# ArtoriasAbyssslayer/HashModNFFBanks-IDR

Hardware: AMD Instinct MI355X
Metric: rays/sec fwd+bwd (hash+SDF MLP) (higher is better)
Workload: dtype f32; 1 GPU; DTU-shaped synthetic uniform-sphere rays, MultiResHash L=16 T=2^19 F=2 (BASELINE.json configs[1]), full IDR training step (forward + IDRLoss + backward + clip + Adam), weights held at the geometric initialisation (lr = 0): the SURVEY.md 8(d) workload; grid_config=C2, rays_per_gpu=2048, global_rays=2048, parallelism=single GPU, world=1, ranks_seen=1, step=HIP-graph captured static-shape step

## Files before the change

### hashmodnffbanks_idr_amd/_lib.py

```python
import ctypes as C
import os

import torch

_PKG = os.path.dirname(os.path.abspath(__file__))
LIB_PATH = os.environ.get("HM_LIB_PATH") or os.path.join(_PKG, "libhashmod.so")
_lib = None

_p = C.c_void_p
_i64 = C.c_int64
_int = C.c_int

SIGNATURES = {
    "hm_version": (_int, []),
    "hm_last_error": (C.c_char_p, []),
    "hm_device_count": (_int, []),
    "hm_grid_desc_create": (_int, [_int, _int, _p, _p, _p, C.POINTER(_p)]),
    "hm_grid_desc_destroy": (None, [_p]),
    "hm_grid_embed_dim": (_int, [_p]),
    "hm_corner_ids": (_int, [_p, _int, _p, _i64, _p, _p, _p]),
    "hm_diag_gather_calib": (_int, [_p, _i64, _i64, _int, _int, _p, _p]),
    "hm_diag_mfma_f32_stream": (_int, [_int, _int, _p, _p]),
    "hm_encode_fwd": (_int, [_p, _p, _i64, _p, _p, _p, _i64, _int, _p]),
    "hm_encode_workspace_bytes": (_i64, [_p, _i64]),
# ... 60 lines not shown
    "hm_gemm_f32_det": (_int, [_int, _int, _i64, _i64, _i64, _p, _i64, _p, _i64, _p, _p, _i64, _int, _p, _i64, _p]),
    "hm_gemm_f32_group_tn_det_workspace_bytes": (_i64, [_p, _int]),
    "hm_gemm_f32_group_tn_det": (_int, [_p, _int, _p, _i64, _p]),
    "hm_gemm_f32_group_tn_add": (_int, [_p, _int, _p]),
    "hm_gemm_f32_group_tn_add_det_workspace_bytes": (_i64, [_p, _int]),
    "hm_gemm_f32_group_tn_add_det": (_int, [_p, _int, _p, _i64, _p]),
    "hm_colsum_det_workspace_bytes": (_i64, [_i64, _i64]),
    "hm_colsum_det": (_int, [_p, _i64, _i64, _i64, _p, _p, _i64, _p]),
    "hm_colsum_acc_det": (_int, [_p, _i64, _i64, _i64, _p, _p, _i64, _p]),
    "hm_colsum_acc_multi_det_workspace_bytes": (_i64, [_p, _int]),
    "hm_colsum_acc_multi_det": (_int, [_p, _int, _p, _i64, _p]),
    "hm_encode_bwd_table_sorted_tracked": (_int, [_p, _p, _p, _i64, _int, _p, _i64, _p, _p, _p, _p, _p, _i64, _p]),
    "hm_gemm_f32_ep": (_int, [_int, _int, _i64, _i64, _i64, _p, _i64, _p, _i64, _p, _p, _i64, _p, _p]),
    "hm_gemm_f32": (_int, [_int, _int, _i64, _i64, _i64, _p, _i64, _p, _i64, _p, _p, _i64, _int, _p]),
    "hm_diag_gemm_plan": (_int, [_int, _int, _i64, _i64, _i64, _p, _i64, _p, _i64, _int, _int, _p]),
    "hm_mc_workspace_bytes": (_i64, [_i64, _i64, _i64]),
    "hm_mc_count": (_int, [_p, _i64, _i64, _i64, _i64, _i64, _i64, C.c_float, _p, _i64, _p, _p]),
    "hm_mc_emit": (_int, [_p, _i64, _i64, _i64, _i64, _i64, _i64, C.c_float, _p, _p, _i64, _i64, _i64, _p, _p, _p,
                          _p]),
    "hm_mcs_points_bricks": (_int, [_p, _i64, _p, _p, _p, _i64, _i64, _i64, _p, _p, _p]),
    "hm_mcs_points_index": (_int, [_p, _i64, _p, _p, _p, _i64, _i64, _i64, _p, _p, _p]),
    "hm_mcs_status": (_int, [_p, _i64, _p, C.c_float, _p, _p]),
    "hm_mcs_workspace_bytes": (_i64, [_i64]),
    "hm_mcs_count": (_int, [_p, _i64, _p, C.c_float, _p, _i64, _p, _p]),
    "hm_mcs_emit": (_int, [_p, _i64, _p, _p, C.c_float, _p, _p, _i64, _i64, _i64, _p, _p, _p, _p, _p, _p]),
    "hm_mesh_cc_labels": (_int, [_p, _i64, _i64, _p, _p, _p]),
    "hm_mesh_cc_face_stats": (_int, [_p, _p, _i64, _i64, _p, _p, _p, _p]),
    "hm_mesh_cc_sums_workspace_bytes": (_i64, [_i64]),
    "hm_mesh_cc_sums": (_int, [_p, _i64, _i64, _p, _p, _p, _i64, _p, _p, _p, _i64, _p, _p]),
    "hm_mesh_moments_workspace_bytes": (_i64, [_i64]),
# ... 247 lines not shown
```

### hashmodnffbanks_idr_amd/csrc/hm_gemm.hip

```cpp
#include "hm_common.h"

namespace {

typedef float f32x16 __attribute__((ext_vector_type(16)));


struct GemmArgs {
    const float *A, *B, *bias;
    float *C;
    int32_t M, N, K;
    int32_t transA, transB;
    int32_t vec_out;
    int64_t lda, ldb, ldc;
    int32_t k_chunk;
    int32_t atomic;
    int32_t vecA, vecB;
    int32_t nrecA, nrecB;
    hm_gemm_epilogue ep;
};

template <int ROWS>
__device__ __forceinline__ int lds_slot(int kg, int row) {
    return (kg * ROWS + (row ^ (kg & 7))) * 4;
}
// ... 420 lines not shown
        const int kg = 2 * oo + h;
        xa[oo] = *reinterpret_cast<const float4 *>(as + lds_slot<AROWS>(kg, arow));
        xb[oo] = *reinterpret_cast<const float4 *>(bs + lds_slot<64>(kg, brow));
    }
}
__device__ __forceinline__ void pipe_mfma_oct(const float4 &a, const float4 &b, f32x16 &c) {
    c = __builtin_amdgcn_mfma_f32_32x32x2f32(a.x, b.x, c, 0, 0, 0);
    c = __builtin_amdgcn_mfma_f32_32x32x2f32(a.y, b.y, c, 0, 0, 0);
    c = __builtin_amdgcn_mfma_f32_32x32x2f32(a.z, b.z, c, 0, 0, 0);
    c = __builtin_amdgcn_mfma_f32_32x32x2f32(a.w, b.w, c, 0, 0, 0);
}


template <bool AKC, bool BKC, bool EP, int WM = 2, bool PART = false, bool KT = false, int ADD = 0>
__device__ __forceinline__ void gemm_pipe2_body(const GemmArgs &g, int bx, int by, int bz, const GemmAddend *ad = nullptr) {
    constexpr int BM = 32 * WM, BN = 64, BK = kPipeBK, NT = 256 * WM, NTB = 512, PER = BM * BK / 4 / NT, KG = BK / 4,
                  OCT = BK / 8 / 2;
    static_assert(PER == 1 && BN * BK / 4 / NTB == 1, "one k-group per thread and operand");
    __shared__ __align__(16) float As_static[ADD ? 1 : 2][ADD ? 4 : BK * BM];
    __shared__ __align__(16) float Bs_static[ADD ? 1 : 2][ADD ? 4 : BK * BN];
    float (*As)[BK * BM], (*Bs)[BK * BN];
    if constexpr (ADD != 0) {
        extern __shared__ __align__(16) float hm_pipe_dyn_lds[];
        As = reinterpret_cast<float (*)[BK * BM]>(hm_pipe_dyn_lds);
        Bs = reinterpret_cast<float (*)[BK * BN]>(hm_pipe_dyn_lds + 2 * BK * BM);
    } else {
        As = As_static;
        Bs = Bs_static;
    }
    const int tid = threadIdx.x;
    const int wave = tid >> 6, lane = tid & 63;
    const int kpart = wave / (2 * WM), wsub = wave % (2 * WM);
    const int wm = wsub >> 1, wn = wsub & 1;
    const int j = lane & 31, h = lane >> 5;
    const int m0 = bx * BM, n0 = by * BN;
    const int kbeg = bz * g.k_chunk;
    const int stages = g.k_chunk / BK;
#ifdef HM_GEMM_PHASE_PROBE
    unsigned long long probe_wait = 0;
#endif
    HM_GEMM_STAMP(0);

    const __amdgpu_buffer_rsrc_t rsA = __builtin_amdgcn_make_buffer_rsrc(const_cast<float *>(g.A), 0, g.nrecA, 0x00020000);
    const __amdgpu_buffer_rsrc_t rsB = __builtin_amdgcn_make_buffer_rsrc(const_cast<float *>(g.B), 0, g.nrecB, 0x00020000);
    int va[PER], vb[PER];
    int kla[PER], klb[PER];
#pragma unroll
    for (int i = 0; i < PER; ++i) {
        const int e = tid + NT * i;
        const int eb = (tid % NTB) + NTB * i;
        const int am = min(m0 + (AKC ? e / KG : e % BM), g.M - 1), bn = min(n0 + (BKC ? eb / KG : eb % BN), g.N - 1);
        va[i] = (int)(4 * (AKC ? (int64_t)am * g.lda + kbeg + (e % KG) * 4
                               : (int64_t)(kbeg + (e / BM) * 4) * g.lda + am));
        vb[i] = (int)(4 * (BKC ? (int64_t)bn * g.ldb + kbeg + (eb % KG) * 4
                               : (int64_t)(kbeg + (eb / BN) * 4) * g.ldb + bn));
        if (KT) {
            kla[i] = g.K - kbeg - (e % KG) * 4;
            klb[i] = g.K - kbeg - (eb % KG) * 4;
        }
    }
    __amdgpu_buffer_rsrc_t rsA2 = rsA, rsB2 = rsB;
    int va2[PER], vb2[PER];
    int sa2 = 0, sb2 = 0, lda24 = 0, ldb24 = 0;
    if constexpr (ADD != 0) {
        static_assert(!AKC && !BKC && !KT, "addends are built for the grouped TN form");
        rsA2 = __builtin_amdgcn_make_buffer_rsrc(const_cast<float *>(ad->A2), 0, ad->nrecA2, 0x00020000);
        rsB2 = __builtin_amdgcn_make_buffer_rsrc(const_cast<float *>(ad->B2), 0, ad->nrecB2, 0x00020000);
        lda24 = 4 * ad->lda2;
        ldb24 = 4 * ad->ldb2;
        sa2 = BK * lda24;
        sb2 = BK * ldb24;
#pragma unroll
        for (int i = 0; i < PER; ++i) {
            const int e = tid + NT * i;
            const int eb = (tid % NTB) + NTB * i;
            const int am = min(m0 + e % BM, g.M - 1), bn = min(n0 + eb % BN, g.N - 1);
            va2[i] = 4 * ((kbeg + (e / BM) * 4 - ad->a_k0) * ad->lda2 + am);
            vb2[i] = 4 * ((kbeg + (eb / BN) * 4 - ad->b_k0) * ad->ldb2 + bn);
        }
    }
#define HM_PIPE_MASK(S_, N_)                                                                        \
    do {                                                                                            \
        if (KT) {                                                                                   \
            pipe_mask_tail<AKC, PER>(ra##N_, kla, (S_) * BK);                                       \
            pipe_mask_tail<BKC, PER>(rb##N_, klb, (S_) * BK);                                       \
        }                                                                                           \
        if constexpr ((ADD & 1) != 0) pipe_add<PER>(ra##N_, qa##N_);                                \
        if constexpr ((ADD & 2) != 0) pipe_add<PER>(rb##N_, qb##N_);                                \
    } while (0)
    const bool stage_b = NT == NTB || tid < NTB;
    const int sa = 4 * (AKC ? BK : BK * (int)g.lda), sb = 4 * (BKC ? BK : BK * (int)g.ldb);
    const int lda4 = 4 * (int)g.lda, ldb4 = 4 * (int)g.ldb;
    f32x16 acc, acc2;
#pragma unroll
    for (int r = 0; r < 16; ++r) acc[r] = acc2[r] = 0.0f;
    static_assert(kPipeD == 4, "the stage macro below is written out for a 4-deep ring (8-deep measured no faster)");
    float4 ra0[PER], ra1[PER], ra2[PER], ra3[PER], rb0[PER], rb1[PER], rb2[PER], rb3[PER];
    float4 qa0[PER], qa1[PER], qa2[PER], qa3[PER], qb0[PER], qb1[PER], qb2[PER], qb3[PER];
    float4 opa0[OCT], opa1[OCT], opb0[OCT], opb1[OCT];
#define HM_PIPE_FETCH(S_, F_)                                                                       \
    do {                                                                                            \
        const int sc_ = min((S_), stages - 1);  \
        pipe_fetch_buf<AKC, PER>(rsA, va, sc_ * sa, lda4, ra##F_);                                  \
        pipe_fetch_buf<BKC, PER>(rsB, vb, sc_ * sb, ldb4, rb##F_);                                  \
        if constexpr ((ADD & 1) != 0) pipe_fetch_add<PER>(rsA2, va2, sc_ * sa2, lda24, qa##F_);     \
        if constexpr ((ADD & 2) != 0) pipe_fetch_add<PER>(rsB2, vb2, sc_ * sb2, ldb24, qb##F_);     \
    } while (0)
    HM_PIPE_FETCH(0, 0);
    HM_PIPE_FETCH(1, 1);
    HM_PIPE_FETCH(2, 2);
    HM_PIPE_MASK(0, 0);
    store_tile<BM, BK, NT>(As[0], AKC, tid, ra0);
    if (stage_b) store_tile<BN, BK, NTB>(Bs[0], BKC, tid, rb0);
    __syncthreads();
    HM_GEMM_STAMP(1);
    pipe_read_ops<OCT, BM>(As[0], Bs[0], wm * 32 + j, wn * 32 + j, h + 4 * kpart, opa0, opb0);
#define HM_PIPE_STAGE(S_, F_, N_, C_, X_, NB_)                                                      \
    do {                                                                                            \
        HM_PIPE_FETCH((S_) + kPipeD - 1, F_);                                                       \
        pipe_mfma_oct(opa##C_[0], opb##C_[0], acc);                                                 \
        HM_PIPE_MASK((S_) + 1, N_);                                                                 \
// ... 71 lines not shown
template <bool AKC, bool BKC, bool EP>
__global__ __launch_bounds__(512, 4) void gemm_f32_pipe2_ktail_kernel(GemmArgs g) {
    gemm_pipe2_body<AKC, BKC, EP, 2, false, true>(g, blockIdx.x, blockIdx.y, blockIdx.z);
}
template <bool AKC, bool BKC, bool EP>
__global__ __launch_bounds__(768, 3) void gemm_f32_pipe2_m96_ktail_kernel(GemmArgs g) {
    gemm_pipe2_body<AKC, BKC, EP, 3, false, true>(g, blockIdx.x, blockIdx.y, blockIdx.z);
}
template <bool AKC, bool BKC>
__global__ __launch_bounds__(512, 4) void gemm_f32_pipe2_part_kernel(GemmArgs g) {
    gemm_pipe2_body<AKC, BKC, false, 2, true>(g, blockIdx.x, blockIdx.y, blockIdx.z);
}
template <bool AKC, bool BKC>
__global__ __launch_bounds__(768, 3) void gemm_f32_pipe2_m96_part_kernel(GemmArgs g) {
    gemm_pipe2_body<AKC, BKC, false, 3, true>(g, blockIdx.x, blockIdx.y, blockIdx.z);
}

struct GemmGroupEntry {
    const float *A, *B;
    float *C;
    int64_t lda, ldb, ldc;
    int32_t M, N, k_chunk, tiles_m, tiles_n, split;
};
struct GemmGroupTable {
    GemmGroupEntry e[HM_GEMM_GROUP_MAX];
    int32_t start[HM_GEMM_GROUP_MAX + 1];
    int32_t n;
};
struct GemmGroupAddTable {
    GemmGroupTable t;
// ... 129 lines not shown
}

static bool gemm_vec_out(const GemmArgs &g, bool part) {
    auto ok = [](const void *p, int64_t ld) { return (reinterpret_cast<uintptr_t>(p) & 15u) == 0 && ld % 4 == 0; };
    if ((g.atomic && !part) || g.N % 4 != 0 || !ok(g.C, g.ldc)) return false;
    const hm_gemm_epilogue &e = g.ep;
    if (e.mode == HM_EPI_NONE) return true;
    const bool masked = e.mode == HM_EPI_S1MUL || e.mode == HM_EPI_RELUMASK;
    const bool has_z = masked || e.mode == HM_EPI_ADJOINT;
    if (!ok(e.out1, e.ld1) || (masked && e.nz % 4 != 0)) return false;
    if (has_z && (!ok(e.z, e.ldz) || (e.g && !ok(e.g, e.ldg)))) return false;
    if (e.mode == HM_EPI_ADJOINT && (!ok(e.out2, e.ld2) || (e.out3 && !ok(e.out3, e.ld3)))) return false;
    return true;
}

static int64_t gemm_det_bytes(const GemmPlan &P, int64_t M, int64_t N) {
    return P.split > 1 ? 4 * P.split * M * N : 0;
}

static int launch_part_reduce(const GemmReduceTable &t, hipStream_t st) {
    if (t.end == 0) return HM_OK;
    HM_CHECK_ARG((t.end + 255) / 256 < (1ll << 31), "hm_gemm_f32_det: too many elements for one reduce launch");
    hipLaunchKernelGGL(gemm_part_reduce_kernel, dim3((unsigned)((t.end + 255) / 256)), dim3(256), 0, st, t);
    return HM_OK;
}

static int gemm_impl(int transA, int transB, int64_t M, int64_t N, int64_t K, const float *A, int64_t lda,
                     const float *B, int64_t ldb, const float *bias, float *C, int64_t ldc, int accumulate,
                     const hm_gemm_epilogue *ep, void *stream, bool det = false, float *ws = nullptr,
                     int64_t ws_bytes = 0) {
    HM_CHECK_ARG(M >= 0 && N >= 0 && K >= 0, "hm_gemm_f32: negative dimension");
    HM_CHECK_ARG(M < (1ll << 31) && N < (1ll << 31) && K < (1ll << 31), "hm_gemm_f32: dimension too large");
    if (M == 0 || N == 0) return HM_OK;
    HM_CHECK_ARG(C != nullptr || (ep && ep->mode != HM_EPI_NONE), "hm_gemm_f32: C is NULL");
    HM_CHECK_ARG(K == 0 || (A && B), "hm_gemm_f32: NULL operand");
    HM_CHECK_ARG(lda >= (transA ? M : K) && ldb >= (transB ? K : N) && (!C || ldc >= N), "hm_gemm_f32: leading dimension");
    GemmArgs g;
    g.ep = hm_gemm_epilogue{};
    if (ep && ep->mode != HM_EPI_NONE) {
        HM_CHECK_ARG(!accumulate, "hm_gemm_f32_ep: an epilogue cannot be combined with accumulate");
        HM_CHECK_ARG(ep->mode >= HM_EPI_SOFTPLUS && ep->mode <= HM_EPI_RELUMASK, "hm_gemm_f32_ep: unknown epilogue mode");
        const bool masked = ep->mode == HM_EPI_S1MUL || ep->mode == HM_EPI_RELUMASK;
        HM_CHECK_ARG(ep->out1 && ep->ld1 >= (masked ? ep->nz : N), "hm_gemm_f32_ep: out1");
        if (ep->mode != HM_EPI_SOFTPLUS && ep->mode != HM_EPI_RELU) {
            const int64_t nzc = masked ? ep->nz : N;
// ... 6 lines not shown
        }
        g.ep = *ep;
    }
    g.A = A; g.B = B; g.bias = bias; g.C = C;
    g.M = (int)M; g.N = (int)N; g.K = (int)K;
    g.transA = transA; g.transB = transB;
    g.lda = lda; g.ldb = ldb; g.ldc = ldc;
    const GemmPlan P = gemm_plan(transA, transB, M, N, K, A, lda, B, ldb, g.ep.mode != HM_EPI_NONE);
    g.vecA = P.vecA ? 1 : 0;
    g.vecB = P.vecB ? 1 : 0;
    const bool big = P.big, m96 = P.m96, pipe_ok = P.pipe_ok;
    const int64_t bm = P.bm, bn = P.bn, split = P.split;
    g.nrecA = (int32_t)(P.bytesA < 0x7fffffff ? P.bytesA : 0x7fffffff);
    g.nrecB = (int32_t)(P.bytesB < 0x7fffffff ? P.bytesB : 0x7fffffff);
    g.k_chunk = (int)P.k_chunk;
    const bool part = det && split > 1;
    if (part) {
        HM_CHECK_ARG(ws != nullptr && ws_bytes >= gemm_det_bytes(P, M, N), "hm_gemm_f32_det: workspace too small");
        g.C = ws;
        g.ldc = N;
    }
    g.atomic = (accumulate || split > 1) ? 1 : 0;
    g.vec_out = gemm_vec_out(g, part) ? 1 : 0;
    if (split > 1 && !accumulate && !part) {
        hipLaunchKernelGGL(zero_window_kernel, dim3((unsigned)((M * N + 255) / 256)), dim3(256), 0, as_stream(stream),
                           C, ldc, M, N);
    }
    dim3 grid((unsigned)((M + bm - 1) / bm), (unsigned)((N + bn - 1) / bn), (unsigned)split);
    HM_CHECK_ARG(grid.y <= 65535u && grid.z <= 65535u, "hm_gemm_f32: N or split too large for one launch");
    hipStream_t st = as_stream(stream);
// ... 66 lines not shown
    HM_CHECK_ARG(M >= 0 && N >= 0 && K >= 0, "hm_diag_gemm_plan: negative dimension");
    *info = hm_gemm_plan_info{};
    if (M == 0 || N == 0) return HM_OK;
    const GemmPlan P = gemm_plan(transA, transB, M, N, K, A, lda, B, ldb, has_epilogue != 0);
    info->kernel = P.big ? HM_GEMM_KERNEL_BIG
                 : P.pipe_ok ? (P.m96 ? HM_GEMM_KERNEL_PIPE96 : HM_GEMM_KERNEL_PIPE64) : HM_GEMM_KERNEL_GENERIC;
    info->k_tail = P.k_tail ? 1 : 0;
    info->vec_a = P.vecA ? 1 : 0;
    info->vec_b = P.vecB ? 1 : 0;
    info->part = (deterministic && P.split > 1) ? 1 : 0;
    info->split = P.split;
    info->k_chunk = P.k_chunk;
    return HM_OK;
}

int hm_gemm_f32_det(int transA, int transB, int64_t M, int64_t N, int64_t K, const float *A, int64_t lda,
                    const float *B, int64_t ldb, const float *bias, float *C, int64_t ldc, int accumulate,
                    void *workspace, int64_t workspace_bytes, void *stream) {
    return gemm_impl(transA, transB, M, N, K, A, lda, B, ldb, bias, C, ldc, accumulate, nullptr, stream, true,
                     static_cast<float *>(workspace), workspace_bytes);
}

}

template <class Item>
static int group_tn(const char *who, const Item *items, int n_items, bool det, float *ws, int64_t ws_bytes,
                    void *stream, bool run, int64_t *need) {
    constexpr bool ADD = std::is_same<Item, hm_gemm_group_add_item>::value;
    HM_CHECK_ARG(n_items >= 0 && (n_items == 0 || items), std::string(who) + ": bad argument");
    *need = 0;
// ... 167 lines not shown
}

#ifdef HM_GEMM_PHASE_PROBE
HM_API int hm_gemm_probe_read(unsigned long long *out, int n) {
    return hipMemcpyFromSymbol(out, HIP_SYMBOL(hm_gemm_probe_ts), sizeof(unsigned long long) * (size_t)(n < 8 ? n : 8)) == hipSuccess ? 0 : -1;
}
#endif

int hm_gemm_f32_ep(int transA, int transB, int64_t M, int64_t N, int64_t K, const float *A, int64_t lda,
                   const float *B, int64_t ldb, const float *bias, float *C, int64_t ldc,
                   const hm_gemm_epilogue *ep, void *stream) {
    HM_CHECK_ARG(ep != nullptr, "hm_gemm_f32_ep: epilogue is NULL");
    return gemm_impl(transA, transB, M, N, K, A, lda, B, ldb, bias, C, ldc, 0, ep, stream);
}

}
```

### hashmodnffbanks_idr_amd/mlp_grad.py

```python
import math

import torch

from . import ops
from .ops import (EPI_ADJOINT, EPI_RELU, EPI_RELUMASK, EPI_S1MUL, EPI_SOFTPLUS, _softplus_call, colsum_into_multi, gemm,
                  gemm_ep, gemm_group_tn, gemm_group_tn_add)

_SQRT2 = math.sqrt(2.0)


class _SdfMlp(torch.autograd.Function):

    @staticmethod
    def forward(ctx, e, skip_layer, beta_sp, thr_sp, beta_rho, cache_out, *params):
        L = len(params) // 2
        Ws, bs = params[:L], params[L:]
        N, E = e.shape
        new = lambda r, c: torch.empty((r, c), dtype=torch.float32, device=e.device)
        stack = [new(2 * N, Ws[l].shape[1]) for l in range(L - 1)] + [None]
        lower = lambda l: stack[l][N:] if stack[l] is not None else None
        a_list, z_list = [], []
        h = None
        for l in range(L):
            if l == 0:
                a = e if stack[0] is None else ops.dcopy_(lower(0), e)
            elif l == skip_layer:
                a = torch.cat([h, e], 1, out=lower(l)).div_(_SQRT2) if stack[l] is not None \
                    else torch.cat([h, e], 1) / _SQRT2
            else:
                a = h
            if l < L - 1:
                dst = lower(l + 1) if (l + 1 != skip_layer and stack[l + 1] is not None) else None
                z, h = gemm_ep(a, Ws[l], bs[l], False, True, EPI_SOFTPLUS, beta_sp, thr_sp, out1=dst)
            else:
                z = gemm(a, Ws[l], bs[l], False, True)
            a_list.append(a)
            z_list.append(z)
        out, sdf, c, denom = ops.sdf_head_fwd(z_list[-1], beta_rho)

        v_list = [None] * L
        v = c.unsqueeze(-1) * Ws[L - 1][0:1, :]
        ge_skip = None
        if skip_layer == L - 1:
            v = v.div_(_SQRT2)
            dh = z_list[L - 2].shape[1]
            ge_skip = v[:, dh:]
            v = v[:, :dh].contiguous()
        v_list[L - 1] = v
        u = _softplus_call(1, z_list[L - 2], v, None, beta_sp, thr_sp)[0] if L > 1 else None
        for l in range(L - 2, -1, -1):
            scale = 1.0 / _SQRT2 if l == skip_layer else 1.0
            if l > 0:
                dh = z_list[l - 1].shape[1]
                v, u = gemm_ep(u, Ws[l], None, False, False, EPI_S1MUL, beta_sp, thr_sp, scale=scale,
                               z=z_list[l - 1], nz=dh)
            else:
                v = gemm(u, Ws[l], None, False, False)
                dh = v.shape[1]
            if l == skip_layer:
                ge_skip = v[:, dh:]
                v = v[:, :dh]
            v_list[l] = v
        g_e = v_list[0] if ge_skip is None else v_list[0] + ge_skip

        ctx.meta = (L, skip_layer, beta_sp, thr_sp, E)
        ctx.stack = stack
        ctx.save_for_backward(e, sdf, c, denom, *Ws, *a_list, *z_list, *v_list)
        ctx.shared = cache_out
        if cache_out is not None:
            cache_out.update(meta=ctx.meta, out=out, g_e=g_e, sdf=sdf, c=c, denom=denom, a_list=a_list, z_list=z_list,
                             v_list=v_list, Ws=Ws,
                             need=(tuple(ctx.needs_input_grad[6:6 + L]), tuple(ctx.needs_input_grad[6 + L:6 + 2 * L])))
# ... 56 lines not shown
            elif stacked and vb_h.data_ptr() != stack[l].data_ptr():
                vb = ops.dcopy_(stack[l][:N], vb_h)
            else:
                vb = vb_h
            if l < L - 1:
                if stacked:
                    ustack[l] = new(2 * N, Ws[l].shape[0])
                nxt = l + 1
                dst = stack[nxt][:N] if (use_stack and nxt < L - 1 and nxt != skip_layer and need_w[nxt]) else None
                loose = (not stacked) and bool(need_w[l])
                if loose and merge:
                    cot[l] = [vb, None]
                    loose = False
                vb_h, zx[l], u_l = gemm_ep(vb, Ws[l], None, False, True, EPI_ADJOINT, beta_sp, thr_sp,
                                           z=z_list[l], g=v_list[l + 1], out1=dst,
                                           out3=ustack[l][:N] if stacked else None, want_out3=loose)
                if loose:
                    wgrad.append((u_l, vb, dW[l]))
            else:
                cb = gemm(vb, Ws[l][0:1], None, False, True)
                if need_w[l]:
                    gemm(c.reshape(N, 1), vb, None, True, False, out=dW[l][0:1], accumulate=True)

    zb = ops.sdf_head_bwd(d_out, sdf, c, denom, cb)
    de = None
    for l in range(L - 1, -1, -1):
        if need_w[l]:
            if l in cot:
                cot[l][1] = zb
            elif ustack[l] is not None:
                if pend is not None and l in pend[2]:
# ... 3 lines not shown
                    wgrad.append((ustack[l], stack[l], dW[l]))
            else:
                wgrad.append((zb, a_list[l], dW[l]))
        if need_b[l]:
            bgrad.append((zb, db[l]))
        if l > 0:
            dh = z_list[l - 1].shape[1]
            is_skip = l == skip_layer
            dst = ustack[l - 1][N:] if ustack[l - 1] is not None else None
            ab, zb = gemm_ep(zb, Ws[l], None, False, False, EPI_S1MUL, beta_sp, thr_sp,
                             scale=1.0 / _SQRT2 if is_skip else 1.0, z=z_list[l - 1], g=zx[l - 1], nz=dh,
                             want_c=is_skip, out1=dst)
            if is_skip:
                de = ab[:, dh:] if de is None else de + ab[:, dh:]
        else:
            ab = gemm(zb, Ws[l], None, False, False)
            de = ab if de is None else de + ab
    if pend is not None and pend[2]:
        raise RuntimeError("hashmod: a _SdfMlpRows node left cotangents for weight gradients this pass does not form")
    if any(len(w) == 5 for w in wgrad):
        gemm_group_tn_add([w if len(w) == 5 else (*w, None, None) for w in wgrad])
    else:
        gemm_group_tn(wgrad)
    colsum_into_multi(bgrad)
    d_e = de if need_e else None
    if cot:
        shared["row_cot"] = (rows[0], rows[1], cot)
    if shared is not None and not owner:
        shared["wgrad_acc"] = (dW, db, (tuple(bool(w) for w in need_w), tuple(bool(b) for b in need_b)))
        return (d_e, *([None] * (2 * L)))
    return (d_e, *dW, *db)
# ... 38 lines not shown
def sdf_mlp_rows(e2, cache, row0, n, weights, biases, merge_wgrad=True):
    ops.require_gpu(e2)
    if e2.shape[0] != n or row0 < 0 or row0 + n > cache["out"].shape[0]:
        raise ValueError("hashmod sdf_mlp_rows: row range does not match")
    return _SdfMlpRows.apply(e2.contiguous(), cache, int(row0), int(n), bool(merge_wgrad), *weights, *biases)


class _ReluMlp(torch.autograd.Function):

    @staticmethod
    def forward(ctx, x, *params):
        L = len(params) // 2
        Ws, bs = params[:L], params[L:]
        acts = [x.contiguous()]
        for l in range(L - 1):
            acts.append(gemm_ep(acts[-1], Ws[l], bs[l], False, True, EPI_RELU, 0.0, 0.0, want_c=False)[1])
        y = gemm(acts[-1], Ws[L - 1], bs[L - 1], False, True)
        ctx.L = L
        ctx.save_for_backward(*Ws, *acts)
        return y

    @staticmethod
    @torch.autograd.function.once_differentiable
    def backward(ctx, d_y):
        L = ctx.L
        sv = ctx.saved_tensors
        Ws, acts = sv[:L], sv[L:]
        need_w = ctx.needs_input_grad[1:1 + L]
        need_b = ctx.needs_input_grad[1 + L:1 + 2 * L]
        dW = [torch.empty_like(Ws[l]) if need_w[l] else None for l in range(L)]
        db = [torch.empty(Ws[l].shape[0], dtype=torch.float32, device=d_y.device) if need_b[l] else None
              for l in range(L)]
        zero_list = [t for t in dW + db if t is not None]
        if zero_list:
            torch._foreach_zero_(zero_list)
        zb = d_y.contiguous()
        dx = None
        wgrad, bgrad = [], []
        for l in range(L - 1, -1, -1):
            if need_w[l]:
                wgrad.append((zb, acts[l], dW[l]))
            if need_b[l]:
                bgrad.append((zb, db[l]))
            if l > 0:
                zb = gemm_ep(zb, Ws[l], None, False, False, EPI_RELUMASK, 0.0, 0.0, z=acts[l], want_c=False)[1]
            elif ctx.needs_input_grad[0]:
                dx = gemm(zb, Ws[0], None, False, False)
        gemm_group_tn(wgrad)
        colsum_into_multi(bgrad)
        return (dx, *dW, *db)


def relu_mlp(x, weights, biases):
    ops.require_gpu(x)
    return _ReluMlp.apply(x, *weights, *biases)
```

### hashmodnffbanks_idr_amd/ops.py

```python
import ctypes as C
import math
from collections import namedtuple

import numpy as np
import torch

from . import _lib
from ._lib import check, dptr, lib, require_gpu, stream_ptr

FRAC_MODES = {"reference": 0, "trilinear": 1}
TILE64_QUARTER = 1664


_DETERMINISTIC = []


class deterministic:

    def __init__(self, enabled=True):
        self.enabled = bool(enabled)

    def __enter__(self):
        _DETERMINISTIC.append(self.enabled)
        return self
# ... 283 lines not shown
    return _HashFeatures.apply(_prep_x(x).detach(), table, B, desc, frac_mode, collector)


def _check_gemm_out(buf, M, cols, dev, what):
    if buf.dtype != torch.float32 or tuple(buf.shape) != (M, cols) or buf.device != dev or \
            (cols > 1 and buf.stride(1) != 1):
        raise ValueError(f"hashmod {what}: bad output buffer (need fp32 [{M}, {cols}] with unit column stride on {dev}; "
                         f"got {buf.dtype} {tuple(buf.shape)} strides {tuple(buf.stride())} on {buf.device})")


def _check_gemm_bias(bias, N, dev, what):
    if bias is not None and (bias.dtype != torch.float32 or bias.numel() != N or bias.device != dev):
        raise ValueError(f"hashmod {what}: bias must be fp32 with N = {N} elements on {dev}")


def gemm(a, b, bias=None, trans_a=False, trans_b=False, out=None, accumulate=False):
    require_gpu(a, b, bias, out)
    if a.dtype != torch.float32 or b.dtype != torch.float32:
        raise TypeError("hashmod gemm: fp32 only")
    M, K = (a.shape[1], a.shape[0]) if trans_a else (a.shape[0], a.shape[1])
    Kb, N = (b.shape[1], b.shape[0]) if trans_b else (b.shape[0], b.shape[1])
    if K != Kb:
        raise ValueError(f"hashmod gemm: inner dimensions differ ({K} vs {Kb})")
    _check_gemm_bias(bias, N, a.device, "gemm")
    if out is not None:
        _check_gemm_out(out, M, N, a.device, "gemm")
    elif accumulate:
        raise ValueError("hashmod gemm: accumulate=True adds into out, which is missing")
    if a.stride(-1) != 1:
        a = a.contiguous()
    if b.stride(-1) != 1:
        b = b.contiguous()
    if out is None:
        out = torch.empty((M, N), dtype=torch.float32, device=a.device)
    if bias is not None:
        bias = bias.contiguous()
    if is_deterministic():
        need = check(lib().hm_gemm_f32_det_workspace_bytes(int(trans_a), int(trans_b), M, N, K, _ld(a), _ld(b)))
        ws, nb = _det_workspace(a.device, need)
        check(lib().hm_gemm_f32_det(int(trans_a), int(trans_b), M, N, K, dptr(a), _ld(a), dptr(b), _ld(b), dptr(bias),
                                    dptr(out), _ld(out), int(accumulate), ws, nb, stream_ptr(a)))
        return out
    check(lib().hm_gemm_f32(int(trans_a), int(trans_b), M, N, K, dptr(a), _ld(a), dptr(b), _ld(b), dptr(bias),
                            dptr(out), _ld(out), int(accumulate), stream_ptr(a)))
    return out


def gemm_group_tn(problems):
    if not problems:
        return
    items = (_lib.GemmGroupItem * len(problems))()
    keep = []
    for i, (a, b, c) in enumerate(problems):
        require_gpu(a, b, c)
        a, b = _rowmajor(a), _rowmajor(b)
        if c.stride(-1) != 1 or a.dtype != torch.float32 or b.dtype != torch.float32 or c.dtype != torch.float32:
            raise ValueError("hashmod gemm_group_tn: fp32 row-major operands expected")
        K, M = a.shape
        Kb, N = b.shape
# ... 58 lines not shown
    check(lib().hm_gemm_f32_group_tn_add(C.cast(items, C.c_void_p), len(problems), stream_ptr(dev)))


EPI_SOFTPLUS, EPI_S1MUL, EPI_ADJOINT, EPI_RELU, EPI_RELUMASK = 1, 2, 3, 4, 5


def _rowmajor(t):
    return t if t.stride(-1) == 1 else t.contiguous()


def _ld(t):
    return t.stride(0) if t.shape[0] > 1 else max(t.stride(0), t.shape[1], 1)


def gemm_ep(a, b, bias, trans_a, trans_b, mode, beta, thr, scale=1.0, z=None, g=None, nz=None, want_c=True,
            want_out3=False, out1=None, out3=None):
    require_gpu(a, b, bias, z, g)
    a, b = _rowmajor(a), _rowmajor(b)
    M, K = (a.shape[1], a.shape[0]) if trans_a else (a.shape[0], a.shape[1])
    Kb, N = (b.shape[1], b.shape[0]) if trans_b else (b.shape[0], b.shape[1])
    if K != Kb:
        raise ValueError(f"hashmod gemm: inner dimensions differ ({K} vs {Kb})")
    dev = a.device
    _check_gemm_bias(bias, N, dev, "gemm_ep")
    new = lambda cols: torch.empty((M, cols), dtype=torch.float32, device=dev)
    ep = _lib.GemmEpilogue()
    ep.mode, ep.scale, ep.beta, ep.threshold = mode, float(scale), float(beta), float(thr)
    c = new(N) if (want_c or mode == EPI_SOFTPLUS) else None
    masked = mode in (EPI_S1MUL, EPI_RELUMASK)
    outs = ()
    def dest(buf, cols):
# ... 16 lines not shown
        if g is not None:
            ep.g, ep.ldg = g.data_ptr(), _ld(g)
        o1 = dest(out1, ncol)
        if masked:
            outs = (c, o1)
        else:
            o2 = new(N)
            o3 = dest(out3, N) if (want_out3 or out3 is not None) else None
            ep.out2, ep.ld2 = o2.data_ptr(), _ld(o2)
            if o3 is not None:
                ep.out3, ep.ld3 = o3.data_ptr(), _ld(o3)
            outs = (o1, o2, o3)
    ep.out1, ep.ld1 = o1.data_ptr(), _ld(o1)
    if bias is not None:
        bias = bias.contiguous()
    check(lib().hm_gemm_f32_ep(int(trans_a), int(trans_b), M, N, K, dptr(a), _ld(a), dptr(b), _ld(b), dptr(bias),
                               dptr(c), _ld(c) if c is not None else N, C.byref(ep), stream_ptr(a)))
    return outs


_INPUT_GRAD_ONLY = [False]


class input_grad_only:

    def __enter__(self):
        self.prev = _INPUT_GRAD_ONLY[0]
        _INPUT_GRAD_ONLY[0] = True

    def __exit__(self, *exc):
        _INPUT_GRAD_ONLY[0] = self.prev

# ... 2186 lines not shown
```

### include/hashmod.h

```cpp
#ifndef HASHMOD_H
#define HASHMOD_H

#include <stdint.h>

#ifdef __cplusplus
extern "C" {
#endif

#if defined(__GNUC__)
#define HM_API __attribute__((visibility("default")))
#else
#define HM_API
#endif

#define HM_MAX_LEVELS 32
#define HM_MAX_LAYERS 16

#define HM_FRAC_REFERENCE 0
#define HM_FRAC_TRILINEAR 1

#define HM_OK 0
#define HM_ERR_INVALID (-1)
#define HM_ERR_HIP (-2)

// ... 226 lines not shown
                          const hm_gemm_epilogue *ep, void *stream);

enum { HM_GEMM_KERNEL_NONE = 0, HM_GEMM_KERNEL_GENERIC = 1, HM_GEMM_KERNEL_BIG = 2, HM_GEMM_KERNEL_PIPE64 = 3,
       HM_GEMM_KERNEL_PIPE96 = 4 };
typedef struct hm_gemm_plan_info {
    int32_t kernel;
    int32_t k_tail;
    int32_t vec_a, vec_b;
    int32_t part;
    int32_t pad_;
    int64_t split, k_chunk;
} hm_gemm_plan_info;
HM_API int hm_diag_gemm_plan(int transA, int transB, int64_t M, int64_t N, int64_t K, const float *A, int64_t lda,
                             const float *B, int64_t ldb, int has_epilogue, int deterministic, hm_gemm_plan_info *info);

HM_API int hm_softplus(int order, const float *z, const float *gy, const float *gg, float *out0, float *out1,
                       int64_t n, float beta, float threshold, void *stream);

typedef struct hm_wn_layer {
    const float *v;
    const float *g;
    float *w;
    float *norm;
    const float *grad_w;
    float *grad_v;
    float *grad_g;
    int32_t rows, cols;
} hm_wn_layer;
HM_API int hm_weight_norm_multi(int backward, int n_layers, const hm_wn_layer *layers, void *stream);

// ... 286 lines not shown
```

Measured before the change: 333,400 rays/s.

## Route short-K epilogue and thin NN GEMMs to new small-tile kernels

Adds a single-pass short-K MFMA kernel (32x64 tiles, 128 threads, no split-K) for NT epilogue GEMMs whose K is at most 384 and that do not qualify for the pipelined path. It also adds a 32-row variant of the pipelined kernel for thin NN GEMMs with N up to 320. The SDF MLP forward and backward opt into both routes. The aim is more blocks and no split-K or atomic overhead on the small MLP GEMMs at 2048 rays, at the cost of more routing logic and new kernels that the existing paths do not cover.

```diff
diff --git a/hashmodnffbanks_idr_amd/_lib.py b/hashmodnffbanks_idr_amd/_lib.py
--- a/hashmodnffbanks_idr_amd/_lib.py
+++ b/hashmodnffbanks_idr_amd/_lib.py
@@ -98,6 +98,9 @@
     "hm_gemm_f32_ep": (_int, [_int, _int, _i64, _i64, _i64, _p, _i64, _p, _i64, _p, _p, _i64, _p, _p]),
     "hm_gemm_f32": (_int, [_int, _int, _i64, _i64, _i64, _p, _i64, _p, _i64, _p, _p, _i64, _int, _p]),
     "hm_diag_gemm_plan": (_int, [_int, _int, _i64, _i64, _i64, _p, _i64, _p, _i64, _int, _int, _p]),
+    "hm_gemm_f32_ep_shortk": (_int, [_int, _int, _i64, _i64, _i64, _p, _i64, _p, _i64, _p, _p, _i64, _p, _p]),
+    "hm_gemm_f32_thin": (_int, [_int, _int, _i64, _i64, _i64, _p, _i64, _p, _i64, _p, _p, _i64, _int, _p]),
+    "hm_diag_gemm_route": (_int, [_int, _int, _i64, _i64, _i64, _i64, _i64, _int, _int, _int]),
     "hm_mc_workspace_bytes": (_i64, [_i64, _i64, _i64]),
     "hm_mc_count": (_int, [_p, _i64, _i64, _i64, _i64, _i64, _i64, C.c_float, _p, _i64, _p, _p]),
     "hm_mc_emit": (_int, [_p, _i64, _i64, _i64, _i64, _i64, _i64, C.c_float, _p, _p, _i64, _i64, _i64, _p, _p, _p,
diff --git a/hashmodnffbanks_idr_amd/csrc/hm_gemm.hip b/hashmodnffbanks_idr_amd/csrc/hm_gemm.hip
--- a/hashmodnffbanks_idr_amd/csrc/hm_gemm.hip
+++ b/hashmodnffbanks_idr_amd/csrc/hm_gemm.hip
@@ -458,9 +458,10 @@
 
 template <bool AKC, bool BKC, bool EP, int WM = 2, bool PART = false, bool KT = false, int ADD = 0>
 __device__ __forceinline__ void gemm_pipe2_body(const GemmArgs &g, int bx, int by, int bz, const GemmAddend *ad = nullptr) {
-    constexpr int BM = 32 * WM, BN = 64, BK = kPipeBK, NT = 256 * WM, NTB = 512, PER = BM * BK / 4 / NT, KG = BK / 4,
-                  OCT = BK / 8 / 2;
-    static_assert(PER == 1 && BN * BK / 4 / NTB == 1, "one k-group per thread and operand");
+    constexpr int BM = 32 * WM, BN = 64, BK = kPipeBK, NT = 256 * WM, NTB = WM == 1 ? 256 : 512, PER = BM * BK / 4 / NT,
+                  PERB = BN * BK / 4 / NTB, KG = BK / 4, OCT = BK / 8 / 2;
+    static_assert(PER == 1 && PERB == (WM == 1 ? 2 : 1), "one k-group per thread and operand (WM = 1: two of B)");
+    static_assert(ADD == 0 || WM != 1, "the addend rings are built for one k-group of B per thread");
     __shared__ __align__(16) float As_static[ADD ? 1 : 2][ADD ? 4 : BK * BM];
     __shared__ __align__(16) float Bs_static[ADD ? 1 : 2][ADD ? 4 : BK * BN];
     float (*As)[BK * BM], (*Bs)[BK * BN];
@@ -487,24 +488,25 @@
 
     const __amdgpu_buffer_rsrc_t rsA = __builtin_amdgcn_make_buffer_rsrc(const_cast<float *>(g.A), 0, g.nrecA, 0x00020000);
     const __amdgpu_buffer_rsrc_t rsB = __builtin_amdgcn_make_buffer_rsrc(const_cast<float *>(g.B), 0, g.nrecB, 0x00020000);
-    int va[PER], vb[PER];
-    int kla[PER], klb[PER];
-#pragma unroll
-    for (int i = 0; i < PER; ++i) {
-        const int e = tid + NT * i;
+    int va[PER], vb[PERB];
+    int kla[PER], klb[PERB];
+#pragma unroll
+    for (int i = 0; i < PERB; ++i) {
+        const int e = tid + NT * (i < PER ? i : 0);
         const int eb = (tid % NTB) + NTB * i;
         const int am = min(m0 + (AKC ? e / KG : e % BM), g.M - 1), bn = min(n0 + (BKC ? eb / KG : eb % BN), g.N - 1);
-        va[i] = (int)(4 * (AKC ? (int64_t)am * g.lda + kbeg + (e % KG) * 4
-                               : (int64_t)(kbeg + (e / BM) * 4) * g.lda + am));
+        if (i < PER)
+            va[i] = (int)(4 * (AKC ? (int64_t)am * g.lda + kbeg + (e % KG) * 4
+                                   : (int64_t)(kbeg + (e / BM) * 4) * g.lda + am));
         vb[i] = (int)(4 * (BKC ? (int64_t)bn * g.ldb + kbeg + (eb % KG) * 4
                                : (int64_t)(kbeg + (eb / BN) * 4) * g.ldb + bn));
         if (KT) {
-            kla[i] = g.K - kbeg - (e % KG) * 4;
+            if (i < PER) kla[i] = g.K - kbeg - (e % KG) * 4;
             klb[i] = g.K - kbeg - (eb % KG) * 4;
         }
     }
     __amdgpu_buffer_rsrc_t rsA2 = rsA, rsB2 = rsB;
-    int va2[PER], vb2[PER];
+    int va2[PER], vb2[PERB];
     int sa2 = 0, sb2 = 0, lda24 = 0, ldb24 = 0;
     if constexpr (ADD != 0) {
         static_assert(!AKC && !BKC && !KT, "addends are built for the grouped TN form");
@@ -527,10 +529,10 @@
     do {                                                                                            \
         if (KT) {                                                                                   \
             pipe_mask_tail<AKC, PER>(ra##N_, kla, (S_) * BK);                                       \
-            pipe_mask_tail<BKC, PER>(rb##N_, klb, (S_) * BK);                                       \
+            pipe_mask_tail<BKC, PERB>(rb##N_, klb, (S_) * BK);                                       \
         }                                                                                           \
         if constexpr ((ADD & 1) != 0) pipe_add<PER>(ra##N_, qa##N_);                                \
-        if constexpr ((ADD & 2) != 0) pipe_add<PER>(rb##N_, qb##N_);                                \
+        if constexpr ((ADD & 2) != 0) pipe_add<PERB>(rb##N_, qb##N_);                                \
     } while (0)
     const bool stage_b = NT == NTB || tid < NTB;
     const int sa = 4 * (AKC ? BK : BK * (int)g.lda), sb = 4 * (BKC ? BK : BK * (int)g.ldb);
@@ -539,16 +541,16 @@
 #pragma unroll
     for (int r = 0; r < 16; ++r) acc[r] = acc2[r] = 0.0f;
     static_assert(kPipeD == 4, "the stage macro below is written out for a 4-deep ring (8-deep measured no faster)");
-    float4 ra0[PER], ra1[PER], ra2[PER], ra3[PER], rb0[PER], rb1[PER], rb2[PER], rb3[PER];
-    float4 qa0[PER], qa1[PER], qa2[PER], qa3[PER], qb0[PER], qb1[PER], qb2[PER], qb3[PER];
+    float4 ra0[PER], ra1[PER], ra2[PER], ra3[PER], rb0[PERB], rb1[PERB], rb2[PERB], rb3[PERB];
+    float4 qa0[PER], qa1[PER], qa2[PER], qa3[PER], qb0[PERB], qb1[PERB], qb2[PERB], qb3[PERB];
     float4 opa0[OCT], opa1[OCT], opb0[OCT], opb1[OCT];
 #define HM_PIPE_FETCH(S_, F_)                                                                       \
     do {                                                                                            \
         const int sc_ = min((S_), stages - 1);  \
         pipe_fetch_buf<AKC, PER>(rsA, va, sc_ * sa, lda4, ra##F_);                                  \
-        pipe_fetch_buf<BKC, PER>(rsB, vb, sc_ * sb, ldb4, rb##F_);                                  \
+        pipe_fetch_buf<BKC, PERB>(rsB, vb, sc_ * sb, ldb4, rb##F_);                                  \
         if constexpr ((ADD & 1) != 0) pipe_fetch_add<PER>(rsA2, va2, sc_ * sa2, lda24, qa##F_);     \
-        if constexpr ((ADD & 2) != 0) pipe_fetch_add<PER>(rsB2, vb2, sc_ * sb2, ldb24, qb##F_);     \
+        if constexpr ((ADD & 2) != 0) pipe_fetch_add<PERB>(rsB2, vb2, sc_ * sb2, ldb24, qb##F_);     \
     } while (0)
     HM_PIPE_FETCH(0, 0);
     HM_PIPE_FETCH(1, 1);
@@ -650,6 +652,101 @@
 template <bool AKC, bool BKC>
 __global__ __launch_bounds__(768, 3) void gemm_f32_pipe2_m96_part_kernel(GemmArgs g) {
     gemm_pipe2_body<AKC, BKC, false, 3, true>(g, blockIdx.x, blockIdx.y, blockIdx.z);
+}
+template <bool AKC, bool BKC>
+__global__ __launch_bounds__(256, 4) void gemm_f32_pipe2_m32_kernel(GemmArgs g) {
+    gemm_pipe2_body<AKC, BKC, false, 1>(g, blockIdx.x, blockIdx.y, blockIdx.z);
+}
+
+constexpr int kShortKMax = 384;
+__global__ __launch_bounds__(128) void gemm_f32_shortk_kernel(GemmArgs g) {
+    constexpr int BM = 32, BN = 64, BK = 128, NT = 128, KG = BK / 4, PA = BM * KG / NT, PB = BN * KG / NT;
+    __shared__ __align__(16) float As[BK * BM];
+    __shared__ __align__(16) float Bs[BK * BN];
+    const int tid = threadIdx.x;
+    const int wn = tid >> 6, lane = tid & 63;
+    const int j = lane & 31, h = lane >> 5;
+    const int m0 = blockIdx.x * BM, n0 = blockIdx.y * BN;
+    const __amdgpu_buffer_rsrc_t rsA = __builtin_amdgcn_make_buffer_rsrc(const_cast<float *>(g.A), 0, g.nrecA, 0x00020000);
+    const __amdgpu_buffer_rsrc_t rsB = __builtin_amdgcn_make_buffer_rsrc(const_cast<float *>(g.B), 0, g.nrecB, 0x00020000);
+    const int kq = (tid % KG) * 4, r0 = tid / KG;
+    int va[PA], vb[PB];
+#pragma unroll
+    for (int i = 0; i < PA; ++i) va[i] = (int)(4 * ((int64_t)min(m0 + r0 + (NT / KG) * i, g.M - 1) * g.lda + kq));
+#pragma unroll
+    for (int i = 0; i < PB; ++i) vb[i] = (int)(4 * ((int64_t)min(n0 + r0 + (NT / KG) * i, g.N - 1) * g.ldb + kq));
+    float4 ra[PA], rb[PB];
+    auto fetch = [&](int b) {
+        const bool in = kq + BK * b < g.K;
+        int oa[PA], ob[PB];
+#pragma unroll
+        for (int i = 0; i < PA; ++i) oa[i] = in ? va[i] + 4 * BK * b : g.nrecA;
+#pragma unroll
+        for (int i = 0; i < PB; ++i) ob[i] = in ? vb[i] + 4 * BK * b : g.nrecB;
+        pipe_fetch_buf<true, PA>(rsA, oa, 0, 0, ra);
+        pipe_fetch_buf<true, PB>(rsB, ob, 0, 0, rb);
+    };
+    f32x16 acc0, acc1;
+#pragma unroll
+    for (int r = 0; r < 16; ++r) acc0[r] = acc1[r] = 0.0f;
+    const int nblk = (g.K + BK - 1) / BK;
+    fetch(0);
+    for (int b = 0; b < nblk; ++b) {
+        if (b > 0) __syncthreads();
+        int kl[PA], klb[PB];
+#pragma unroll
+        for (int i = 0; i < PA; ++i) kl[i] = g.K - kq;
+#pragma unroll
+        for (int i = 0; i < PB; ++i) klb[i] = g.K - kq;
+        pipe_mask_tail<true, PA>(ra, kl, BK * b);
+        pipe_mask_tail<true, PB>(rb, klb, BK * b);
+        store_tile<BM, BK, NT>(As, true, tid, ra);
+        store_tile<BN, BK, NT>(Bs, true, tid, rb);
+        __syncthreads();
+        fetch(b + 1);
+        const int rem = g.K - BK * b;
+        const int n0c = min(8, (rem + 7) / 8), n1c = min(8, max(0, (rem - 64 + 7) / 8));
+        for (int oo = 0; oo < n0c; ++oo) {
+            const int kg = 2 * oo + h;
+            pipe_mfma_oct(*reinterpret_cast<const float4 *>(As + lds_slot<BM>(kg, j)),
+                          *reinterpret_cast<const float4 *>(Bs + lds_slot<BN>(kg, wn * 32 + j)), acc0);
+        }
+        for (int oo = 0; oo < n1c; ++oo) {
+            const int kg = 2 * (8 + oo) + h;
+            pipe_mfma_oct(*reinterpret_cast<const float4 *>(As + lds_slot<BM>(kg, j)),
+                          *reinterpret_cast<const float4 *>(Bs + lds_slot<BN>(kg, wn * 32 + j)), acc1);
+        }
+    }
+#pragma unroll
+    for (int r = 0; r < 16; ++r) acc0[r] += acc1[r];
+    __syncthreads();
+    const bool add_bias = g.bias != nullptr;
+    float *const turn = Bs + wn * 512;
+#pragma unroll
+    for (int half = 0; half < 2; ++half) {
+        float fin[8];
+#pragma unroll
+        for (int q = 0; q < 8; ++q) fin[q] = acc0[8 * half + q];
+        if (g.vec_out) {
+            auto slot = [](int row, int col) { return (row >> 1) * 64 + (((row ^ (row >> 2)) & 1) * 32) + col; };
+            __builtin_amdgcn_fence(__ATOMIC_RELEASE, "wavefront");
+            __builtin_amdgcn_wave_barrier();
+#pragma unroll
+            for (int q = 0; q < 8; ++q) turn[slot((q & 3) + 8 * (q >> 2) + 4 * h, j)] = fin[q];
+            __builtin_amdgcn_fence(__ATOMIC_RELEASE, "wavefront");
+            __builtin_amdgcn_wave_barrier();
+            __builtin_amdgcn_fence(__ATOMIC_ACQUIRE, "wavefront");
+            const int row = lane >> 3, col = (lane & 7) * 4;
+            float4 quad[2];
+#pragma unroll
+            for (int i = 0; i < 2; ++i) quad[i] = *reinterpret_cast<const float4 *>(turn + slot(row + 8 * i, col));
+            const int n = n0 + wn * 32 + col;
+            if (n < g.N) gemm_store_quads<true>(g, quad, n, m0 + 16 * half + row, add_bias);
+        } else {
+            const int n = n0 + wn * 32 + j;
+            if (n < g.N) gemm_store_oct<true>(g, fin, n, m0 + 16 * half + 4 * h, add_bias);
+        }
+    }
 }
 
 struct GemmGroupEntry {
@@ -809,6 +906,20 @@
     return true;
 }
 
+static int gemm_route(int transA, int transB, int64_t M, int64_t N, int64_t K, int64_t lda, int64_t ldb, int ep_mode,
+                      bool has_bias, bool accumulate) {
+    if (M <= 0 || N <= 0 || K <= 0 || M >= (1ll << 31) || N >= (1ll << 31) || K >= (1ll << 31) || accumulate)
+        return HM_GEMM_ROUTE_DEFAULT;
+    const GemmPlan P = gemm_plan(transA, transB, M, N, K, nullptr, lda, nullptr, ldb, ep_mode != HM_EPI_NONE);
+    if (P.big || P.bytesA >= (1ll << 31) || P.bytesB >= (1ll << 31)) return HM_GEMM_ROUTE_DEFAULT;
+    const bool short_ep = ep_mode == HM_EPI_SOFTPLUS || ep_mode == HM_EPI_ADJOINT || ep_mode == HM_EPI_RELU;
+    if (!transA && transB && short_ep && !P.pipe_ok && K <= kShortKMax) return HM_GEMM_ROUTE_SHORTK;
+    const int64_t t64 = ((M + 63) / 64) * ((N + 63) / 64);
+    if (!transA && !transB && ep_mode == HM_EPI_NONE && !has_bias && K % (kPipeBK * kPipeD) == 0 && N <= 320 && t64 < 256)
+        return HM_GEMM_ROUTE_THIN;
+    return HM_GEMM_ROUTE_DEFAULT;
+}
+
 static int64_t gemm_det_bytes(const GemmPlan &P, int64_t M, int64_t N) {
     return P.split > 1 ? 4 * P.split * M * N : 0;
 }
@@ -823,7 +934,7 @@
 static int gemm_impl(int transA, int transB, int64_t M, int64_t N, int64_t K, const float *A, int64_t lda,
                      const float *B, int64_t ldb, const float *bias, float *C, int64_t ldc, int accumulate,
                      const hm_gemm_epilogue *ep, void *stream, bool det = false, float *ws = nullptr,
-                     int64_t ws_bytes = 0) {
+                     int64_t ws_bytes = 0, int route_hint = HM_GEMM_ROUTE_DEFAULT) {
     HM_CHECK_ARG(M >= 0 && N >= 0 && K >= 0, "hm_gemm_f32: negative dimension");
     HM_CHECK_ARG(M < (1ll << 31) && N < (1ll << 31) && K < (1ll << 31), "hm_gemm_f32: dimension too large");
     if (M == 0 || N == 0) return HM_OK;
@@ -860,6 +971,22 @@
     g.nrecA = (int32_t)(P.bytesA < 0x7fffffff ? P.bytesA : 0x7fffffff);
     g.nrecB = (int32_t)(P.bytesB < 0x7fffffff ? P.bytesB : 0x7fffffff);
     g.k_chunk = (int)P.k_chunk;
+    if (route_hint != HM_GEMM_ROUTE_DEFAULT &&
+        gemm_route(transA, transB, M, N, K, lda, ldb, g.ep.mode, bias != nullptr, accumulate != 0) == route_hint) {
+        g.k_chunk = (int)K;
+        g.atomic = 0;
+        g.vec_out = gemm_vec_out(g, false) ? 1 : 0;
+        if (route_hint == HM_GEMM_ROUTE_SHORTK) {
+            dim3 grid((unsigned)((M + 31) / 32), (unsigned)((N + 63) / 64));
+            HM_CHECK_ARG(grid.y <= 65535u, "hm_gemm_f32_ep_shortk: N too large for one launch");
+            hipLaunchKernelGGL(gemm_f32_shortk_kernel, grid, dim3(128), 0, as_stream(stream), g);
+        } else {
+            dim3 grid((unsigned)((M + 31) / 32), (unsigned)((N + 63) / 64));
+            hipLaunchKernelGGL((gemm_f32_pipe2_m32_kernel<true, false>), grid, dim3(256), 0, as_stream(stream), g);
+        }
+        HM_CHECK_LAUNCH("hm_gemm_f32");
+        return HM_OK;
+    }
     const bool part = det && split > 1;
     if (part) {
         HM_CHECK_ARG(ws != nullptr && ws_bytes >= gemm_det_bytes(P, M, N), "hm_gemm_f32_det: workspace too small");
@@ -956,6 +1083,18 @@
     return HM_OK;
 }
 
+int hm_gemm_f32_thin(int transA, int transB, int64_t M, int64_t N, int64_t K, const float *A, int64_t lda,
+                     const float *B, int64_t ldb, const float *bias, float *C, int64_t ldc, int accumulate,
+                     void *stream) {
+    return gemm_impl(transA, transB, M, N, K, A, lda, B, ldb, bias, C, ldc, accumulate, nullptr, stream, false, nullptr, 0,
+                     HM_GEMM_ROUTE_THIN);
+}
+
+int hm_diag_gemm_route(int transA, int transB, int64_t M, int64_t N, int64_t K, int64_t lda, int64_t ldb,
+                       int epilogue_mode, int has_bias, int accumulate) {
+    return gemm_route(transA, transB, M, N, K, lda, ldb, epilogue_mode, has_bias != 0, accumulate != 0);
+}
+
 int hm_gemm_f32_det(int transA, int transB, int64_t M, int64_t N, int64_t K, const float *A, int64_t lda,
                     const float *B, int64_t ldb, const float *bias, float *C, int64_t ldc, int accumulate,
                     void *workspace, int64_t workspace_bytes, void *stream) {
@@ -1153,4 +1292,12 @@
     return gemm_impl(transA, transB, M, N, K, A, lda, B, ldb, bias, C, ldc, 0, ep, stream);
 }
 
-}
+int hm_gemm_f32_ep_shortk(int transA, int transB, int64_t M, int64_t N, int64_t K, const float *A, int64_t lda,
+                          const float *B, int64_t ldb, const float *bias, float *C, int64_t ldc,
+                          const hm_gemm_epilogue *ep, void *stream) {
+    HM_CHECK_ARG(ep != nullptr, "hm_gemm_f32_ep_shortk: epilogue is NULL");
+    return gemm_impl(transA, transB, M, N, K, A, lda, B, ldb, bias, C, ldc, 0, ep, stream, false, nullptr, 0,
+                     HM_GEMM_ROUTE_SHORTK);
+}
+
+}
diff --git a/hashmodnffbanks_idr_amd/mlp_grad.py b/hashmodnffbanks_idr_amd/mlp_grad.py
--- a/hashmodnffbanks_idr_amd/mlp_grad.py
+++ b/hashmodnffbanks_idr_amd/mlp_grad.py
@@ -31,7 +31,7 @@
                 a = h
             if l < L - 1:
                 dst = lower(l + 1) if (l + 1 != skip_layer and stack[l + 1] is not None) else None
-                z, h = gemm_ep(a, Ws[l], bs[l], False, True, EPI_SOFTPLUS, beta_sp, thr_sp, out1=dst)
+                z, h = gemm_ep(a, Ws[l], bs[l], False, True, EPI_SOFTPLUS, beta_sp, thr_sp, out1=dst, shortk=True)
             else:
                 z = gemm(a, Ws[l], bs[l], False, True)
             a_list.append(a)
@@ -55,7 +55,7 @@
                 v, u = gemm_ep(u, Ws[l], None, False, False, EPI_S1MUL, beta_sp, thr_sp, scale=scale,
                                z=z_list[l - 1], nz=dh)
             else:
-                v = gemm(u, Ws[l], None, False, False)
+                v = gemm(u, Ws[l], None, False, False, thin=True)
                 dh = v.shape[1]
             if l == skip_layer:
                 ge_skip = v[:, dh:]
@@ -142,7 +142,7 @@
                     loose = False
                 vb_h, zx[l], u_l = gemm_ep(vb, Ws[l], None, False, True, EPI_ADJOINT, beta_sp, thr_sp,
                                            z=z_list[l], g=v_list[l + 1], out1=dst,
-                                           out3=ustack[l][:N] if stacked else None, want_out3=loose)
+                                           out3=ustack[l][:N] if stacked else None, want_out3=loose, shortk=True)
                 if loose:
                     wgrad.append((u_l, vb, dW[l]))
             else:
@@ -176,7 +176,7 @@
             if is_skip:
                 de = ab[:, dh:] if de is None else de + ab[:, dh:]
         else:
-            ab = gemm(zb, Ws[l], None, False, False)
+            ab = gemm(zb, Ws[l], None, False, False, thin=True)
             de = ab if de is None else de + ab
     if pend is not None and pend[2]:
         raise RuntimeError("hashmod: a _SdfMlpRows node left cotangents for weight gradients this pass does not form")
@@ -245,7 +245,7 @@
         Ws, bs = params[:L], params[L:]
         acts = [x.contiguous()]
         for l in range(L - 1):
-            acts.append(gemm_ep(acts[-1], Ws[l], bs[l], False, True, EPI_RELU, 0.0, 0.0, want_c=False)[1])
+            acts.append(gemm_ep(acts[-1], Ws[l], bs[l], False, True, EPI_RELU, 0.0, 0.0, want_c=False, shortk=True)[1])
         y = gemm(acts[-1], Ws[L - 1], bs[L - 1], False, True)
         ctx.L = L
         ctx.save_for_backward(*Ws, *acts)
@@ -276,7 +276,7 @@
             if l > 0:
                 zb = gemm_ep(zb, Ws[l], None, False, False, EPI_RELUMASK, 0.0, 0.0, z=acts[l], want_c=False)[1]
             elif ctx.needs_input_grad[0]:
-                dx = gemm(zb, Ws[0], None, False, False)
+                dx = gemm(zb, Ws[0], None, False, False, thin=True)
         gemm_group_tn(wgrad)
         colsum_into_multi(bgrad)
         return (dx, *dW, *db)
diff --git a/hashmodnffbanks_idr_amd/ops.py b/hashmodnffbanks_idr_amd/ops.py
--- a/hashmodnffbanks_idr_amd/ops.py
+++ b/hashmodnffbanks_idr_amd/ops.py
@@ -321,7 +321,7 @@
         raise ValueError(f"hashmod {what}: bias must be fp32 with N = {N} elements on {dev}")
 
 
-def gemm(a, b, bias=None, trans_a=False, trans_b=False, out=None, accumulate=False):
+def gemm(a, b, bias=None, trans_a=False, trans_b=False, out=None, accumulate=False, thin=False):
     require_gpu(a, b, bias, out)
     if a.dtype != torch.float32 or b.dtype != torch.float32:
         raise TypeError("hashmod gemm: fp32 only")
@@ -348,8 +348,9 @@
         check(lib().hm_gemm_f32_det(int(trans_a), int(trans_b), M, N, K, dptr(a), _ld(a), dptr(b), _ld(b), dptr(bias),
                                     dptr(out), _ld(out), int(accumulate), ws, nb, stream_ptr(a)))
         return out
-    check(lib().hm_gemm_f32(int(trans_a), int(trans_b), M, N, K, dptr(a), _ld(a), dptr(b), _ld(b), dptr(bias),
-                            dptr(out), _ld(out), int(accumulate), stream_ptr(a)))
+    call = lib().hm_gemm_f32_thin if thin else lib().hm_gemm_f32
+    check(call(int(trans_a), int(trans_b), M, N, K, dptr(a), _ld(a), dptr(b), _ld(b), dptr(bias),
+               dptr(out), _ld(out), int(accumulate), stream_ptr(a)))
     return out
 
 
@@ -438,7 +439,7 @@
 
 
 def gemm_ep(a, b, bias, trans_a, trans_b, mode, beta, thr, scale=1.0, z=None, g=None, nz=None, want_c=True,
-            want_out3=False, out1=None, out3=None):
+            want_out3=False, out1=None, out3=None, shortk=False):
     require_gpu(a, b, bias, z, g)
     a, b = _rowmajor(a), _rowmajor(b)
     M, K = (a.shape[1], a.shape[0]) if trans_a else (a.shape[0], a.shape[1])
@@ -485,8 +486,9 @@
     ep.out1, ep.ld1 = o1.data_ptr(), _ld(o1)
     if bias is not None:
         bias = bias.contiguous()
-    check(lib().hm_gemm_f32_ep(int(trans_a), int(trans_b), M, N, K, dptr(a), _ld(a), dptr(b), _ld(b), dptr(bias),
-                               dptr(c), _ld(c) if c is not None else N, C.byref(ep), stream_ptr(a)))
+    call = lib().hm_gemm_f32_ep_shortk if shortk else lib().hm_gemm_f32_ep
+    check(call(int(trans_a), int(trans_b), M, N, K, dptr(a), _ld(a), dptr(b), _ld(b), dptr(bias),
+               dptr(c), _ld(c) if c is not None else N, C.byref(ep), stream_ptr(a)))
     return outs
 
 
diff --git a/include/hashmod.h b/include/hashmod.h
--- a/include/hashmod.h
+++ b/include/hashmod.h
@@ -264,6 +264,16 @@
 HM_API int hm_diag_gemm_plan(int transA, int transB, int64_t M, int64_t N, int64_t K, const float *A, int64_t lda,
                              const float *B, int64_t ldb, int has_epilogue, int deterministic, hm_gemm_plan_info *info);
 
+enum { HM_GEMM_ROUTE_DEFAULT = 0, HM_GEMM_ROUTE_SHORTK = 1, HM_GEMM_ROUTE_THIN = 2 };
+HM_API int hm_gemm_f32_ep_shortk(int transA, int transB, int64_t M, int64_t N, int64_t K, const float *A, int64_t lda,
+                                 const float *B, int64_t ldb, const float *bias, float *C, int64_t ldc,
+                                 const hm_gemm_epilogue *ep, void *stream);
+HM_API int hm_gemm_f32_thin(int transA, int transB, int64_t M, int64_t N, int64_t K, const float *A, int64_t lda,
+                            const float *B, int64_t ldb, const float *bias, float *C, int64_t ldc, int accumulate,
+                            void *stream);
+HM_API int hm_diag_gemm_route(int transA, int transB, int64_t M, int64_t N, int64_t K, int64_t lda, int64_t ldb,
+                              int epilogue_mode, int has_bias, int accumulate);
+
 HM_API int hm_softplus(int order, const float *z, const float *gy, const float *gg, float *out0, float *out1,
                        int64_t n, float beta, float threshold, void *stream);
 
```

New measurement: 335,400 rays/s, median of 6. Within noise of the previous version (+0.6%).
